# viscom-ulm/MCCNN

Measured on AMD Instinct MI355X. Metric: MC-convolved points/sec (fwd+bwd), 100k-pt cloud r=0.1, higher is better.
Workload: dtype f32; 1 GPU; ScanNet-like non-uniform room, 100000 pts/room, 1 room(s) on rank 0, absolute radius 0.1, KDE window 0.2, same-level conv 1to64 (Fin=1, Fout=64, combin), avg on; points_total=100000, points_per_gpu=100000, edges_per_gpu=4543198, layer=1to64, parallelism=cloud-per-GPU dp1, headline_mode=pipelined, rccl_world_size=1, collectives_warmed_before_warmup=False

## Files before the change

### mccnn_amd/MCConvModule.py

```python
import ctypes as C
import os
import threading
import time
import weakref

import numpy as _np
import torch

from . import _env, _lib
from ._lib import check, ptr, stream_handle


class InvalidArgumentError(ValueError):
    pass


def _req(cond, msg):
    if not cond:
        raise InvalidArgumentError(msg)


def _f32(t, name):
    _req(isinstance(t, torch.Tensor) and t.is_cuda, "%s must be a CUDA tensor" % name)
    _req(t.dtype == torch.float32, "%s must be float32" % name)
# ... 355 lines not shown
    if e <= 500000:
        return True
    if not backward:
        return not (fin <= 128 and feats.shape[0] >= 65536)
    return fin >= 256 and e / float(rows) >= ROWS_MIN_DEGREE


def clear_caches():
    _ORDER_HINTS.clear()
    _WS_POOL.clear()
    _NUM_CELLS_CACHE.clear()
    _EDGE_GUESS.clear()
    _EDGE_RATIO.clear()


CHECK_BATCH_IDS = False


def check_batch_ids(inBatchIds, batchSize):
    bids = _i32(inBatchIds, "batch_ids")
    bad = torch.empty(1, dtype=torch.int32, device=bids.device)
    check(_lib.load().mccnn_check_batch_ids(ptr(bids), bids.shape[0], int(batchSize), ptr(bad), stream_handle()),
          "check_batch_ids")
    return int(bad.item())


_DEBUG_IMPL = 0


def debug_conv_impl(mask):
    global _DEBUG_IMPL
    prev = _DEBUG_IMPL
    _DEBUG_IMPL = int(mask)
    _lib.load().mccnn_debug_conv_impl(int(mask) & 3)
    return prev


def _num_cells(aabbMin, aabbMax, batchSize, cellSize, scaleInv):
    lib = _lib.load()
    if scaleInv:
        out = C.c_int(0)
        check(lib.mccnn_num_cells(None, None, batchSize, float(cellSize), 1, C.byref(out), None), "num_cells")
        return out.value
    key = (id(aabbMin), id(aabbMax))
    hit = _NUM_CELLS_CACHE.get(key)
    ext = None
    if hit is not None:
        rmin, rmax, vmin, vmax, val = hit
        if rmin() is aabbMin and rmax() is aabbMax and vmin == aabbMin._version and vmax == aabbMax._version:
            ext = val
    if ext is None:
        out = C.c_float(0.0)
        check(lib.mccnn_aabb_extent(ptr(aabbMin), ptr(aabbMax), C.byref(out), stream_handle()), "aabb_extent")
        ext = _np.float32(out.value)
        _evict_oldest(_NUM_CELLS_CACHE, 256)
        _NUM_CELLS_CACHE[key] = (weakref.ref(aabbMin), weakref.ref(aabbMax), aabbMin._version, aabbMax._version, ext)
    _req(cellSize > 0, "cell size must be positive")
    nc = int(ext / _np.float32(cellSize))
    return nc if nc != 0 else 1


def _seed_num_cells(aabbMin, aabbMax, extent):
    _evict_oldest(_NUM_CELLS_CACHE, 256)
    _NUM_CELLS_CACHE[(id(aabbMin), id(aabbMax))] = (weakref.ref(aabbMin), weakref.ref(aabbMax), aabbMin._version,
                                                    aabbMax._version, _np.float32(extent))


# ... 937 lines not shown
```

### mccnn_amd/_env.py

```python
import os
import sys

KNOWN_KEYS = (
    "small_off", "plan_small", "plan_small_max_l", "plan_mid_l", "plan_min_l", "rows_force",
    "rows_min_degree", "unsorted_max_points", "force_valu", "no_f1", "f1_x4_min_e", "f1_x4_waves_per_cu", "nw_lean",
    "nw_lds_pad", "scan_bg_tiles", "issue_thread", "job_delay_us",
    "hier_trace", "geo_own_pool", "trace_terminate", "aabb_one_max", "plan_batch_sync", "caller_join_off", "bwd_min_chunks",
    "fuse_sort", "native_prefetch", "plan_prefetch", "plan_prefetch_max_e", "geo_prefetch_min",
    "ecap_scale", "hier_pmode", "geo_trace")


def _parse():
    out = {}
    for item in os.environ.get("MCCNN_DEBUG", "").split(","):
        item = item.strip()
        if not item:
            continue
        k, _, v = item.partition("=")
        out[k.strip()] = v.strip() if _ else "1"
        if k.strip() not in KNOWN_KEYS:
            sys.stderr.write("mccnn: MCCNN_DEBUG key %r is not known (mccnn_amd/_env.py KNOWN_KEYS): ignored\n" % k.strip())
    return out


_OPTS = _parse()


def flag(name, default=True):
    v = os.environ.get("MCCNN_" + name)
    if v is None:
        return default
    return v != "0"


def debug(key, default, cast=None):
    v = _OPTS.get(key)
    if v is None:
        return default
    if cast is not None:
        return cast(v)
# ... 8 lines not shown
```

### mccnn_amd/csrc/conv.hip

```cpp
#include "conv_mfma.h"
#include "batch.h"
#include <cstdlib>
#include <type_traits>

namespace mccnn {

__device__ __forceinline__ float relu(float x) { return fmaxf(x, 0.0f); }
__device__ __forceinline__ float wave_sum(float v) {
#pragma unroll
    for (int d = 32; d >= 1; d >>= 1) v += __shfl_xor(v, d, 64);
    return v;
}

struct EdgeCtx {
    int j, i;
    float d0, d1, d2, inv;
};

__device__ __forceinline__ EdgeCtx load_edge(const ConvArgs& a, int t) {
    EdgeCtx c;
    int2 pr = a.packed[t];
    c.j = pr.x;
    c.i = pr.y;
    int b = clamp_batch(a.bids[c.j], a.B);
// ... 954 lines not shown
    if ((a.nb * 8) % Fin != 0) return MCCNN_E_SHAPE;
    a.outF = combin ? Fout : Fin;
    a.pts = sorted_pts; a.feats = sorted_feats; a.bids = sorted_batch_ids; a.pdfs = pdfs; a.samples = samples;
    a.start = start_idx; a.packed = reinterpret_cast<const int2*>(packed); a.mn = aabb_min; a.mx = aabb_max;
    a.w1 = w1; a.b1 = b1; a.w2 = w2; a.b2 = b2; a.w3 = w3; a.b3 = b3;
    a.n = n; a.m = m; a.e = e; a.Fin = Fin; a.Fout = Fout; a.radius = radius; a.invRadius = 1.0f / radius; a.scaleInv = scale_inv; a.avg = avg; a.B = batch_size;
    if (m > 0 && (!samples || !start_idx || !aabb_min || !aabb_max || !w1 || !b1 || !w2 || !b2 || !w3 || !b3))
        return MCCNN_E_BADARG;
    if (e > 0 && (!sorted_pts || !sorted_feats || !sorted_batch_ids || !pdfs || !packed)) return MCCNN_E_BADARG;
    return 0;
}

int launch_edge_records(const ConvArgs& a, float4* rec, hipStream_t s) {
    edge_records<<<ceil_div(a.e, 256), 256, 0, s>>>(a, rec);
    MCCNN_LAUNCHED();
    return 0;
}

void launch_reduce_partials(const float* partials, int rows, int nb, float* dw1, float* db1, float* dw2, float* db2,
                            float* dw3, float* db3, hipStream_t s) {
    reduce_partials<<<ceil_div((long long)nb * 176, 16), 1024, 0, s>>>(partials, rows, nb, dw1, db1, dw2, db2, dw3, db3, no_span());
}

int conv_fill_args(ConvArgs& a, const float* sorted_pts, const float* sorted_feats, const int* sorted_batch_ids,
                   const float* pdfs, const float* samples, const int* start_idx, const int* packed,
                   const float* aabb_min, const float* aabb_max, const float* w1, const float* b1, const float* w2,
                   const float* b2, const float* w3, const float* b3, int n, int m, int e, int Fin, int Fout, int combin,
                   int batch_size, float radius, int scale_inv, int avg) {
    return fill_args(a, sorted_pts, sorted_feats, sorted_batch_ids, pdfs, samples, start_idx, packed, aabb_min, aabb_max, w1,
                     b1, w2, b2, w3, b3, n, m, e, Fin, Fout, combin, batch_size, radius, scale_inv, avg);
}

std::atomic<int>& conv_impl_override() {
    static std::atomic<int> v{(debug_int("force_valu", 0) ? 1 : 0) | (debug_int("no_f1", 0) ? 2 : 0)};
    return v;
}

bool transpose_small(int e, int n) {
    return e <= MCCNN_TR_SMALL_E && n <= MCCNN_TR_SMALL_N && (long long)e * e / n <= (1LL << 20) && small_kernels_on();
}
size_t transpose_count_bytes(int n) { return align_up((size_t)n * 4) + scan_workspace_bytes(n); }
int transpose_count(const int2* pk, int e, int n, int* start_t, char* blk, int* slot, hipStream_t s) {
    const size_t cntBytes = align_up((size_t)n * 4);
    int* cnt = (int*)blk;
    {
        int rc = launch_clear_spans(clear_span(blk, cntBytes + scan_status_bytes(n)), no_span(), no_span(), s);
        if (rc) return rc;
    }
    if (n <= MCCNN_TR_LDS_BINS && e >= 4 * n) tr_count_lds<<<ceil_div(e, 256), 256, 0, s>>>(pk, e, n, cnt, slot);
    else tr_count<<<ceil_div(e, 256), 256, 0, s>>>(pk, e, cnt, slot);
    MCCNN_LAUNCHED();
    return exclusive_scan_i32(cnt, start_t, n, start_t + n, blk + cntBytes, s, true);
}
int transpose_fill(const int2* pk, int e, const int* start_t, const int* slot, int* tmp, hipStream_t s) {
    tr_fill<<<ceil_div(e, 256), 256, 0, s>>>(pk, e, start_t, slot, tmp);
    MCCNN_LAUNCHED();
    return 0;
}

}

using namespace mccnn;

template <bool TR>
static int launch_conv_stream(const ConvArgs& a, bool combin, bool vec, bool bf16, float* out, const float4* rec,
                              const int* permT, hipStream_t s, float4* recOut = nullptr) {
    typedef void (*Kern)(ConvArgs, float*, int, const float4*, const int*, float4*);
    Kern fn;
    if (bf16) fn = TR ? conv_stream<false, 4, true> : conv_stream<false, 4, false>;
    else if (TR) fn = vec ? conv_stream<false, 2, true> : conv_stream<false, 0, true>;
    else if (combin) fn = (a.Fin == 1) ? conv_stream<true, 1, false> : (a.Fin <= 4 ? conv_stream<true, 3, false> : conv_stream<true, 0, false>);
    else fn = vec ? conv_stream<false, 2, false> : conv_stream<false, 0, false>;
    const size_t lds = ((size_t)a.nb * MCCNN_WQ_FWD + 4 * (size_t)a.nb * 8) * sizeof(float);
    const int numCU = num_cus();
    const int perCU = cached_blocks_per_cu(reinterpret_cast<const void*>(fn), lds);
    const long long chunks = ((long long)a.e + 63) / 64;
    long long W = (long long)numCU * perCU * 4;
    if (W > (chunks + 1) / 2) W = (chunks + 1) / 2;
    if (W < 1) W = 1;
    fn<<<(int)((W + 3) / 4), 256, lds, s>>>(a, out, (int)W, rec, permT, recOut);
    MCCNN_LAUNCHED();
    return 0;
}

extern "C" {

int mccnn_debug_conv_impl(int mask) { return conv_impl_override().exchange(mask & 3); }

static bool f1_shape(int num_in_feats, int num_out_feats, int combin) {
    return combin && num_in_feats == 1 && num_out_feats > 0 && (num_out_feats + 7) / 8 <= MCCNN_LDS_MAX_NB &&
           (conv_impl_override().load(std::memory_order_relaxed) & 3) == 0;
}

static size_t state_record_bytes(int e) { return align_up((size_t)(e > 0 ? e : 0) * sizeof(float4)); }
size_t mccnn_spatial_conv_state_bytes(int m, int e, int num_in_feats, int num_out_feats, int combin) {
    if (m <= 0 || e <= 0 || num_in_feats <= 0 || num_out_feats <= 0) return 0;
    if (f1_shape(num_in_feats, num_out_feats, combin)) return state_record_bytes(e) + f1_state_bytes(m, (num_out_feats + 7) / 8);
    const long long neurons = combin ? (long long)num_in_feats * num_out_feats : num_in_feats;
    const bool mfma = (!combin || (neurons + 7) / 8 <= MCCNN_LDS_MAX_NB) && (conv_impl_override().load(std::memory_order_relaxed) & 1) == 0;
    return mfma ? state_record_bytes(e) : 0;
}

size_t mccnn_spatial_conv_fwd_workspace_bytes(int m, int e, int num_in_feats, int num_out_feats, int combin) {
    (void)e;
    if (m > 0 && f1_shape(num_in_feats, num_out_feats, combin)) return f1_fwd_workspace_bytes(m, (num_out_feats + 7) / 8);
    return 256;
}

static bool use_mfma(const ConvArgs& a, bool combin) {
    return (a.nb <= MCCNN_LDS_MAX_NB || !combin) && (conv_impl_override().load(std::memory_order_relaxed) & 1) == 0;
}
#define MCCNN_TILE_FWD 64
#define MCCNN_TILE_BWD 48
static void tile_split(int nb, int maxTile, int& tiles, int& per) {
    tiles = (nb + maxTile - 1) / maxTile;
    per = (nb + tiles - 1) / tiles;
}
static ConvArgs tile_args(const ConvArgs& a, int q0, int nbT, size_t elem) {
    ConvArgs t = a;
    t.feats = reinterpret_cast<const float*>(reinterpret_cast<const char*>(a.feats) + (size_t)q0 * 8 * elem);
// ... 336 lines not shown
```

### mccnn_amd/csrc/conv_f1.hip

```cpp
#include "conv_mfma.h"

namespace mccnn {

__device__ __forceinline__ float wave_seg_scan1(float v, float m1, float m2, float m4, float m8, float mA, float mB) {
    asm("s_nop 1\n"
        "v_fmac_f32_dpp %0, %0, %1 row_shr:1 row_mask:0xf bank_mask:0xf bound_ctrl:1\n s_nop 1\n"
        "v_fmac_f32_dpp %0, %0, %2 row_shr:2 row_mask:0xf bank_mask:0xf bound_ctrl:1\n s_nop 1\n"
        "v_fmac_f32_dpp %0, %0, %3 row_shr:4 row_mask:0xf bank_mask:0xf bound_ctrl:1\n s_nop 1\n"
        "v_fmac_f32_dpp %0, %0, %4 row_shr:8 row_mask:0xf bank_mask:0xf bound_ctrl:1\n s_nop 1\n"
        "v_fmac_f32_dpp %0, %0, %5 row_bcast:15 row_mask:0xa bank_mask:0xf\n s_nop 1\n"
        "v_fmac_f32_dpp %0, %0, %6 row_bcast:31 row_mask:0xc bank_mask:0xf\n s_nop 1\n"
        : "+v"(v)
        : "v"(m1), "v"(m2), "v"(m4), "v"(m8), "v"(mA), "v"(mB));
    return v;
}

__global__ __launch_bounds__(256) void f1_fwd_edges(ConvArgs a, float* __restrict__ A, float* __restrict__ S,
                                                    int numWaves, float4* __restrict__ recOut) {
    extern __shared__ float lds[];
    const int wave = threadIdx.x >> 6, lane = threadIdx.x & 63, i4 = lane & 3;
    const int rowA = a.nb * 8;
    float* wl = lds;
    float* carry = lds + a.nb * MCCNN_WQ_FWD + (size_t)wave * rowA;
    stage_weights<MCCNN_WQ_FWD>(a, wl);
// ... 464 lines not shown
                gb2[k] += t3[k];
            }
            float t4[8];
            MCCNN_PHASE();
            layer8<false>(w4 + 46, nullptr, i4, t3, t4);
            MCCNN_PHASE();
#pragma unroll
            for (int l = 0; l < 8; ++l) {
                float v = p1[l] ? t4[l] : 0.f;
                gw1[l * 3] = fmaf(v, rc.x, gw1[l * 3]);
                gw1[l * 3 + 1] = fmaf(v, rc.y, gw1[l * 3 + 1]);
                gw1[l * 3 + 2] = fmaf(v, rc.z, gw1[l * 3 + 2]);
                gb1[l] += v;
            }
        }
        {
            float r2 = wave_reduce64(gw2, lane);
            float misc[64];
#pragma unroll
            for (int k = 0; k < 24; ++k) misc[k] = gw1[k];
#pragma unroll
            for (int k = 0; k < 8; ++k) { misc[24 + k] = gb1[k]; misc[32 + k] = gb2[k]; }
#pragma unroll
            for (int k = 40; k < 64; ++k) misc[k] = 0.f;
            float rm = wave_reduce64(misc, lane);
            float* pq = prow + q * MCCNN_F1_ROW;
            pq[32 + lane] = r2;
            if (lane < 32) pq[lane] = rm;
            else if (lane < 40) pq[96 + lane - 32] = rm;
        }
    }
}

#define MCCNN_F1_ROWC 72
__global__ __launch_bounds__(256) void f1_bwd_centres(ConvArgs a, const float* __restrict__ outGrad,
                                                      const float* __restrict__ A, const float* __restrict__ S,
                                                      int cPerWave, int numSlices, float* __restrict__ G,
                                                      float* __restrict__ gb, float* __restrict__ partials,
                                                      float* __restrict__ featGrad) {
    for (long long i = (long long)blockIdx.x * blockDim.x + threadIdx.x; i < a.n; i += (long long)gridDim.x * blockDim.x)
        featGrad[i] = 0.f;
    const int wave = threadIdx.x >> 6, lane = threadIdx.x & 63;
    const int wid = blockIdx.x * 4 + wave;
    const int w = __builtin_amdgcn_readfirstlane(wid / (a.nb + 1));
    const int q = __builtin_amdgcn_readfirstlane(wid - w * (a.nb + 1));
    if (w >= numSlices) return;
    const int c0 = w * cPerWave;
    const int c1 = min(a.m, c0 + cPerWave);
    if (q == a.nb) {
        for (int i = c0 + lane; i < c1; i += 64) {
            const float* row = outGrad + (size_t)i * a.outF;
            float gbv = 0.f;
            int f = 0;
            if ((a.outF & 3) == 0) {
                for (; f + 4 <= a.outF; f += 4) {
                    const float4 gg = *reinterpret_cast<const float4*>(row + f);
                    gbv = fmaf(gg.x, a.b3[f], gbv);
                    gbv = fmaf(gg.y, a.b3[f + 1], gbv);
                    gbv = fmaf(gg.z, a.b3[f + 2], gbv);
                    gbv = fmaf(gg.w, a.b3[f + 3], gbv);
                }
            }
            for (; f < a.outF; ++f) gbv = fmaf(row[f], a.b3[f], gbv);
            gb[i] = gbv;
        }
        return;
// ... 74 lines not shown
            s2 += src[(size_t)(w + 128) * stride];
            s3 += src[(size_t)(w + 192) * stride];
        }
        for (; w < rows; w += 64) s0 += src[(size_t)w * stride];
    }
    acc[sl][kk] = (s0 + s1) + (s2 + s3);
    __syncthreads();
    if (sl == 0 && k < K) {
        float v = 0.f;
#pragma unroll
        for (int i = 0; i < 64; ++i) v += acc[i][kk];
        if (r < 24) dw1[q * 24 + r] = v;
        else if (r < 32) db1[q * 8 + r - 24] = v;
        else if (r < 96) dw2[q * 64 + r - 32] = v;
        else if (r < 104) db2[q * 8 + r - 96] = v;
        else if (r < 168) dw3[q * 64 + r - 104] = v;
        else db3[q * 8 + r - 168] = v;
    }
}

static void f1_bwd_partition(int e, int& cpw, int& waves) {
    const long long chunks = ((long long)e + 63) / 64;
    const long long resident = (long long)num_cus() * 4 * MCCNN_F1_OCC;
    cpw = (int)((chunks + resident - 1) / resident);
    if (cpw > 48) {
        const long long rounds = (cpw + 31) / 32;
        cpw = (int)((chunks + resident * rounds - 1) / (resident * rounds));
    }
    static const int minChunks = debug_int("bwd_min_chunks", 2);
    if (cpw < minChunks) cpw = minChunks < 1 ? 1 : minChunks;
    waves = (int)((chunks + cpw - 1) / cpw);
    if (waves < 1) waves = 1;
}
#ifndef MCCNN_F1_CENTRE_WAVES
#define MCCNN_F1_CENTRE_WAVES 1024
#endif
static void f1_centre_partition(int m, int& cPerWave, int& waves) {
    cPerWave = (m + MCCNN_F1_CENTRE_WAVES - 1) / MCCNN_F1_CENTRE_WAVES;
    cPerWave = (cPerWave + 63) / 64 * 64;
    waves = (m + cPerWave - 1) / cPerWave;
}

size_t f1_state_bytes(int m, int nb) { return align_up((size_t)m * nb * 8 * sizeof(float)) + align_up((size_t)m * sizeof(float)); }

static void f1_state_split(void* state, int m, int nb, float*& A, float*& S) {
    A = (float*)state;
    S = (float*)((char*)state + align_up((size_t)m * nb * 8 * sizeof(float)));
}

static int f1_run_edges(const ConvArgs& a, float* A, float* S, float4* recOut, hipStream_t s) {
    const size_t lds = ((size_t)a.nb * MCCNN_WQ_FWD + 4 * (size_t)a.nb * 8) * sizeof(float);
    if (a.e >= g_f1_x4_min_edges.load(std::memory_order_relaxed)) {
        const size_t lds4 = lds + 4 * 256 * sizeof(float4);
        const int perCU4 = cached_blocks_per_cu(reinterpret_cast<const void*>(f1_fwd_edges4), lds4);
        const long long iters = ((long long)a.e + 255) / 256;
        static const int wpc = debug_int("f1_x4_waves_per_cu", 0);
        long long W4 = (long long)num_cus() * (wpc > 0 ? wpc : perCU4 * 4);
        if (W4 > (iters + 1) / 2) W4 = (iters + 1) / 2;
        if (W4 < 1) W4 = 1;
        f1_fwd_edges4<<<(int)((W4 + 3) / 4), 256, lds4, s>>>(a, A, S, (int)W4, recOut);
        MCCNN_LAUNCHED();
        return 0;
    }
    const int perCU = cached_blocks_per_cu(reinterpret_cast<const void*>(f1_fwd_edges), lds);
    const long long chunks = ((long long)a.e + 63) / 64;
    long long W = (long long)num_cus() * perCU * 4;
    if (W > (chunks + 1) / 2) W = (chunks + 1) / 2;
    if (W < 1) W = 1;
    f1_fwd_edges<<<(int)((W + 3) / 4), 256, lds, s>>>(a, A, S, (int)W, recOut);
    MCCNN_LAUNCHED();
    return 0;
}

size_t f1_fwd_workspace_bytes(int m, int nb) { return f1_state_bytes(m, nb) + 256; }

int f1_forward(const ConvArgs& a, float* out, float4* rec_out, void* state, void* ws, size_t ws_bytes, hipStream_t s) {
    if (!state) {
        if (!ws || ws_bytes < f1_fwd_workspace_bytes(a.m, a.nb)) return MCCNN_E_WORKSPACE;
        state = ws;
    }
    float *A, *S;
    f1_state_split(state, a.m, a.nb, A, S);
    int rc = f1_run_edges(a, A, S, rec_out, s);
    if (rc) return rc;
    f1_fwd_centres<<<ceil_div((long long)a.m * a.nb, 256), 256, (size_t)a.nb * 72 * sizeof(float), s>>>(a, A, S, out);
    MCCNN_LAUNCHED();
    return 0;
}

size_t f1_bwd_workspace_bytes(int m, int e, int nb) {
    int cpw, wavesE, cpwC, wavesC;
    f1_bwd_partition(e, cpw, wavesE);
    f1_centre_partition(m, cpwC, wavesC);
    size_t b = f1_state_bytes(m, nb);
    b += align_up((size_t)m * nb * 8 * sizeof(float)) + align_up((size_t)m * sizeof(float));
    b += align_up((size_t)e * sizeof(float4)) + align_up((size_t)e * sizeof(float));
    b += align_up((size_t)(wavesE + 3) / 4 * 4 * nb * MCCNN_F1_ROW * sizeof(float));
    b += align_up((size_t)(wavesC + 3) / 4 * 4 * nb * MCCNN_F1_ROWC * sizeof(float));
    return b + 256;
}

int f1_backward(const ConvArgs& a, const float* out_grad, const float4* rec_in, const void* state, float* feat_grad, float* dw1, float* db1,
                float* dw2, float* db2, float* dw3, float* db3, void* ws, size_t ws_bytes, hipStream_t s) {
    if (!ws || ws_bytes < f1_bwd_workspace_bytes(a.m, a.e, a.nb)) return MCCNN_E_WORKSPACE;
    int cpw, wavesE, cPerWave, wavesC;
    f1_bwd_partition(a.e, cpw, wavesE);
    f1_centre_partition(a.m, cPerWave, wavesC);
    const int blocksE = (wavesE + 3) / 4, blocksC = (wavesC + 3) / 4;
    Arena ar(ws, ws_bytes);
    void* own = ar.take<char>(f1_state_bytes(a.m, a.nb));
    float* G = ar.take<float>((size_t)a.m * a.nb * 8);
    float* gb = ar.take<float>((size_t)a.m);
    float4* rec = ar.take<float4>((size_t)a.e);
    float* dfE = ar.take<float>((size_t)a.e);
    float* pe = ar.take<float>((size_t)blocksE * 4 * a.nb * MCCNN_F1_ROW);
    float* pc = ar.take<float>((size_t)blocksC * 4 * a.nb * MCCNN_F1_ROWC);
    if (!own || !G || !gb || !rec || !dfE || !pe || !pc) return MCCNN_E_WORKSPACE;
    float *A, *S;
    if (state) {
        f1_state_split(const_cast<void*>(state), a.m, a.nb, A, S);
    } else {
        f1_state_split(own, a.m, a.nb, A, S);
        int rc = f1_run_edges(a, A, S, nullptr, s);
        if (rc) return rc;
    }
    f1_bwd_centres<<<ceil_div((long long)wavesC * (a.nb + 1), 4), 256, 0, s>>>(a, out_grad, A, S, cPerWave, wavesC, G, gb, pc, feat_grad);
    MCCNN_LAUNCHED();
    const float4* recUse = rec;
    if (rec_in) {
        recUse = rec_in;
    } else {
        f1_edge_records<<<ceil_div(a.e, 256), 256, 0, s>>>(a, rec);
        MCCNN_LAUNCHED();
    }
    const size_t ldsE = (size_t)a.nb * MCCNN_WQ_BWD * sizeof(float);
    f1_bwd_edges<<<blocksE, 256, ldsE, s>>>(a, recUse, G, gb, feat_grad, dfE, cpw, pe);
    MCCNN_LAUNCHED();
    f1_reduce<<<ceil_div((long long)a.nb * 176, 16), 1024, 0, s>>>(pe, wavesE, pc, wavesC, a.nb, dw1, db1, dw2, db2, dw3, db3);
    MCCNN_LAUNCHED();
    return 0;
}

}
```

### mccnn_amd/csrc/conv_mfma.h

```cpp
#pragma once
#include "common.h"
#include <atomic>
#include <mutex>

namespace mccnn {

struct ConvArgs {
    const float* pts;
    const float* feats;
    const int* bids;
    const float* pdfs;
    const float* samples;
    const int* start;
    const int2* packed;
    const float* mn;
    const float* mx;
    const float *w1, *b1, *w2, *b2, *w3, *b3;
    int n, m, e, Fin, Fout, nb, neuronsOut, outF;
    float radius, invRadius;
    int scaleInv, avg, G, B;
};

#define MCCNN_LDS_MAX_NB 64
#define MCCNN_WQ_FWD 184
// ... 59 lines not shown
    if (BIAS) { bl = bias[i4]; bh = bias[4 + i4]; }
    f32x4 lo = {0.f, 0.f, 0.f, 0.f}, hi = lo;
#pragma unroll
    for (int k = 0; k < 8; ++k) {
        lo = MFMA4(al[k], x[k], lo);
        hi = MFMA4(ah[k], x[k], hi);
    }
    if (BIAS) {
        const float one = opaque_one();
        lo = MFMA4(bl, one, lo);
        hi = MFMA4(bh, one, hi);
    }
#pragma unroll
    for (int r = 0; r < 4; ++r) { y[r] = lo[r]; y[4 + r] = hi[r]; }
}

template <bool BIAS>
__device__ __forceinline__ void layer8_regs(const float* al, const float* ah, float bl, float bh, const float* x, float* y) {
    f32x4 lo = {0.f, 0.f, 0.f, 0.f}, hi = lo;
#pragma unroll
    for (int k = 0; k < 8; ++k) {
        lo = MFMA4(al[k], x[k], lo);
        hi = MFMA4(ah[k], x[k], hi);
    }
    if (BIAS) {
        const float one = opaque_one();
        lo = MFMA4(bl, one, lo);
        hi = MFMA4(bh, one, hi);
    }
#pragma unroll
    for (int r = 0; r < 4; ++r) { y[r] = lo[r]; y[4 + r] = hi[r]; }
}

struct BlockWeights {
    float w1lo[4], w1hi[4];
    float w2lo[8], w2hi[8], b2lo, b2hi;
    float w3lo[8], w3hi[8], b3lo, b3hi;
};
__device__ __forceinline__ void load_block_weights(const ConvArgs& a, int q, int i4, BlockWeights& w) {
    const int nl = q * 8 + i4, nh = nl + 4;
#pragma unroll
    for (int c = 0; c < 3; ++c) { w.w1lo[c] = a.w1[nl * 3 + c]; w.w1hi[c] = a.w1[nh * 3 + c]; }
    w.w1lo[3] = a.b1[nl]; w.w1hi[3] = a.b1[nh];
    const float4* r2l = reinterpret_cast<const float4*>(a.w2 + (size_t)q * 64 + i4 * 8);
    const float4* r2h = reinterpret_cast<const float4*>(a.w2 + (size_t)q * 64 + (4 + i4) * 8);
    const float4* r3l = reinterpret_cast<const float4*>(a.w3 + (size_t)q * 64 + i4 * 8);
    const float4* r3h = reinterpret_cast<const float4*>(a.w3 + (size_t)q * 64 + (4 + i4) * 8);
    const float4 a0 = r2l[0], a1 = r2l[1], b0 = r2h[0], b1 = r2h[1], c0 = r3l[0], c1 = r3l[1], d0 = r3h[0], d1 = r3h[1];
    w.w2lo[0] = a0.x; w.w2lo[1] = a0.y; w.w2lo[2] = a0.z; w.w2lo[3] = a0.w; w.w2lo[4] = a1.x; w.w2lo[5] = a1.y; w.w2lo[6] = a1.z; w.w2lo[7] = a1.w;
    w.w2hi[0] = b0.x; w.w2hi[1] = b0.y; w.w2hi[2] = b0.z; w.w2hi[3] = b0.w; w.w2hi[4] = b1.x; w.w2hi[5] = b1.y; w.w2hi[6] = b1.z; w.w2hi[7] = b1.w;
    w.w3lo[0] = c0.x; w.w3lo[1] = c0.y; w.w3lo[2] = c0.z; w.w3lo[3] = c0.w; w.w3lo[4] = c1.x; w.w3lo[5] = c1.y; w.w3lo[6] = c1.z; w.w3lo[7] = c1.w;
    w.w3hi[0] = d0.x; w.w3hi[1] = d0.y; w.w3hi[2] = d0.z; w.w3hi[3] = d0.w; w.w3hi[4] = d1.x; w.w3hi[5] = d1.y; w.w3hi[6] = d1.z; w.w3hi[7] = d1.w;
    w.b2lo = a.b2[nl]; w.b2hi = a.b2[nh];
    w.b3lo = a.b3[nl]; w.b3hi = a.b3[nh];
}
__device__ __forceinline__ void mlp_block_regs(const BlockWeights& w, float d0, float d1, float d2, float* a1, float* a2, float* o) {
    float pre[8];
    {
        f32x4 lo = {0.f, 0.f, 0.f, 0.f}, hi = lo;
        const float one = opaque_one();
        lo = MFMA4(w.w1lo[0], d0, lo);
        hi = MFMA4(w.w1hi[0], d0, hi);
        lo = MFMA4(w.w1lo[1], d1, lo);
        hi = MFMA4(w.w1hi[1], d1, hi);
        lo = MFMA4(w.w1lo[2], d2, lo);
        hi = MFMA4(w.w1hi[2], d2, hi);
        lo = MFMA4(w.w1lo[3], one, lo);
        hi = MFMA4(w.w1hi[3], one, hi);
#pragma unroll
        for (int r = 0; r < 4; ++r) { pre[r] = lo[r]; pre[4 + r] = hi[r]; }
    }
    MCCNN_PHASE();
#pragma unroll
    for (int r = 0; r < 8; ++r) a1[r] = relu1(pre[r]);
    MCCNN_PHASE();
    layer8_regs<true>(w.w2lo, w.w2hi, w.b2lo, w.b2hi, a1, pre);
    MCCNN_PHASE();
#pragma unroll
    for (int r = 0; r < 8; ++r) a2[r] = relu1(pre[r]);
    MCCNN_PHASE();
    layer8_regs<true>(w.w3lo, w.w3hi, w.b3lo, w.b3hi, a2, o);
    MCCNN_PHASE();
}

__device__ __forceinline__ void layer1_mfma(const f32x4* __restrict__ w, int i4, float d0, float d1, float d2, float* pre1) {
    f32x4 a1lo = w[i4], a1hi = w[4 + i4];
    f32x4 lo = {0.f, 0.f, 0.f, 0.f}, hi = lo;
    const float one = opaque_one();
    lo = MFMA4(a1lo.x, d0, lo);
    hi = MFMA4(a1hi.x, d0, hi);
    lo = MFMA4(a1lo.y, d1, lo);
    hi = MFMA4(a1hi.y, d1, hi);
    lo = MFMA4(a1lo.z, d2, lo);
    hi = MFMA4(a1hi.z, d2, hi);
    lo = MFMA4(a1lo.w, one, lo);
    hi = MFMA4(a1hi.w, one, hi);
#pragma unroll
    for (int r = 0; r < 4; ++r) { pre1[r] = lo[r]; pre1[4 + r] = hi[r]; }
}

__device__ __forceinline__ void mlp_block_l12(const float* __restrict__ wq, int i4, float d0, float d1, float d2,
                                              float* pre1, float* a1, float* pre2, float* a2) {
    const f32x4* w = reinterpret_cast<const f32x4*>(wq);
    layer1_mfma(w, i4, d0, d1, d2, pre1);
// ... 241 lines not shown
```

### mccnn_amd/csrc/debug_opts.h

```cpp
#pragma once
#include <cstdio>
#include <cstdlib>
#include <cstring>
#include <string>

namespace mccnn {

#define MCCNN_DEBUG_KEYS                                                                                                   \
    "small_off", "plan_small", "plan_small_max_l", "plan_mid_l", "plan_min_l", "rows_force",                              \
    "rows_min_degree", "unsorted_max_points", "force_valu", "no_f1", "f1_x4_min_e", "f1_x4_waves_per_cu", "nw_lean",      \
    "nw_lds_pad", "scan_bg_tiles", "issue_thread", "job_delay_us",                                                       \
    "hier_trace", "geo_own_pool", "trace_terminate", "aabb_one_max", "plan_batch_sync", "caller_join_off", "bwd_min_chunks", \
                                                                                    \
    "fuse_sort", "native_prefetch", "plan_prefetch", "plan_prefetch_max_e", "geo_prefetch_min",                          \
    "ecap_scale", "hier_pmode", "geo_trace"
static const char* const kDebugKeys[] = {MCCNN_DEBUG_KEYS};

inline const std::string& debug_list() {
    static const std::string list = [] {
        const char* e = getenv("MCCNN_DEBUG");
        std::string l(e ? e : "");
        size_t p = 0;
        while (p < l.size()) {
            size_t q = l.find(',', p);
            if (q == std::string::npos) q = l.size();
            size_t a = p, b = q;
            while (a < b && l[a] == ' ') ++a;
            while (b > a && l[b - 1] == ' ') --b;
            size_t eq = l.find('=', a);
            if (eq == std::string::npos || eq > b) eq = b;
            size_t kb = eq;
            while (kb > a && l[kb - 1] == ' ') --kb;
            const std::string key = l.substr(a, kb - a);
            if (!key.empty()) {
                bool known = false;
                for (const char* k : kDebugKeys) known = known || key == k;
                if (!known) fprintf(stderr, "mccnn: MCCNN_DEBUG key '%s' is not known (csrc/debug_opts.h kDebugKeys): ignored\n", key.c_str());
            }
            p = q + 1;
        }
        return l;
    }();
    return list;
}

// ... 24 lines not shown
```

### mccnn_amd/csrc/exec.hip

```cpp
#include "batch.h"

#include <chrono>
#include <cstdlib>
#include <cstring>
#include <new>
#include <thread>

namespace mccnn {
std::atomic<int>& conv_impl_override();
ClearSpan grid_head_span(int n, int batch_size, int num_cells, void* ws, size_t ws_bytes);
int build_grid_fused(const float* pts, const int* batch_ids, const float* aabb_min, const float* aabb_max, int n,
                     int batch_size, int num_cells, int* new_idx, float* out_pts, int* out_batch_ids, int* cell_indexs,
                     int* inv_idx, void* ws, size_t ws_bytes, hipStream_t s, const int* n_dev, bool cleared, ClearSpan x1,
                     ClearSpan x2);
size_t visiting_order_workspace_bytes(int m, int batch_size, int num_cells);
ClearSpan visiting_order_head_span(int m, int batch_size, int num_cells, void* ws, size_t ws_bytes);
int visiting_order(const float* pts, const int* batch_ids, const float* aabb_min, const float* aabb_max, int m, int batch_size,
                   int num_cells, int* order, void* ws, size_t ws_bytes, hipStream_t s, bool cleared);
bool plan_batchable(int rows, int e, int transposed);
size_t plan_batch_tr_ws_bytes(int n, int e);
int plan_batch_items(int transposed, const float* sorted_pts, const int* sorted_batch_ids, const float* pdfs, const float* samples,
                     const int* start_idx, const int* packed, const float* aabb_min, const float* aabb_max, int n, int m, int e,
                     int batch_size, float radius, int scale_inv, int avg, const int* order, int* start_t, int* perm_t,
                     int tlist_ready, void* plan_buffer, void* tws, size_t tws_bytes, TrSmallItem* tr, bool* use_tr,
// ... 77 lines not shown
        L.cells = o; o += al(cells_of(B, nc) * 8);
        L.new_idx = o; o += al(n1 * 4);
        L.inv_idx = o; o += al(n1 * 4);
    }
    L.start = o; o += al(m1 * 4);
    L.packed = o; o += al(e1 * 8);
    L.pdfs = o; o += al(e1 * 4);
    L.total = o; o += 256;
    L.order = o; o += al(m1 * 4);
    size_t w = mccnn_find_neighbors_workspace_bytes(m, n);
    size_t head = 0;
    if (with_grid) {
        const size_t g = mccnn_build_grid_workspace_bytes(n, B, nc);
        if (g == 0) return L;
        head += al(g);
    }
    if (m >= MCCNN_ORDER_MIN_M) {
        const size_t c = visiting_order_workspace_bytes(m, B, nc);
        if (c == 0) return L;
        head += al(c);
    }
    if (head > w) w = head;
    if (mccnn_sort_step1_workspace_bytes(m, B, nc) == 0) return L;
    const size_t p = mccnn_compute_pdf_workspace_bytes(e_cap, 1);
    if (p > w) w = p;
    if (max_neighbors > 0) w = al(w) + (mccnn_find_neighbors_capped_workspace_bytes(m, n) - mccnn_find_neighbors_workspace_bytes(m, n));
    L.ws = o;
    L.ws_bytes = al(w) + 256;
    o += L.ws_bytes;
    L.total_bytes = o;
    return L;
}

int read_mask() { return conv_impl_override().load(std::memory_order_relaxed); }

bool env_flag(const char* name, bool dflt) {
    const char* v = getenv(name);
    return v ? (strcmp(v, "0") != 0) : dflt;
}
bool row_kernels_on() { static const bool on = env_flag("MCCNN_ROW_KERNELS", true); return on; }
float rows_min_degree() { static const float d = (float)debug_float("rows_min_degree", 16.0); return d; }
int unsorted_max_points() { static const int v = debug_int("unsorted_max_points", 32768); return v; }

bool rows_shape(bool combin, int fin, const void* feats, int rows, int n_points, int e, bool backward) {
    if (!row_kernels_on() || read_mask() != 0 || combin || fin % 8 != 0 || e <= 0 || rows <= 0 || (((uintptr_t)feats) & 15)) return false;
    static const int force = debug_int("rows_force", 0);
    if (force == 1) return true;
    if (e <= 500000) return true;
    if (!backward) return !(fin <= 128 && n_points >= 65536);
    return fin >= 256 && (float)e / (float)rows >= rows_min_degree();
}

std::atomic<long long> g_wait_ns{0};

thread_local bool t_count_waits = true;

int wait_edges(mccnn_geometry* g, int spin_us) {
    if (g->e >= 0) return g->e;
    if (!g->total_host) return -1;
    int v = *g->total_host;
    if (v < 0 && spin_us != 0) {
        const auto t0 = std::chrono::steady_clock::now();
        struct Acc {
            std::chrono::steady_clock::time_point t;
            ~Acc() { if (t_count_waits) g_wait_ns.fetch_add(std::chrono::duration_cast<std::chrono::nanoseconds>(std::chrono::steady_clock::now() - t).count(), std::memory_order_relaxed); }
        } acc{t0};
        for (;;) {
// ... 972 lines not shown
```

Baseline: 171.8 million points/s.

## Add cooperative multi-wave F1 backward edge kernel sharing edge sweeps across waves

Adds a cooperative backward edge kernel for the Fin=1 combin path. W waves in a block each own one output-feature block per sweep, process the same edge chunk, and exchange per-edge feature-gradient partial sums through a small LDS buffer, so each edge's gradient accumulation is done cooperatively instead of each wave redoing it. It is selected when the edge count covers enough chunks per resident group. It also adds a per-edge barrier and extra register pressure from the per-wave gradient accumulators, and it repartitions the partials buffer. New debug mask bits control the path, and read_mask is masked so other code ignores them.

```diff
diff --git a/mccnn_amd/MCConvModule.py b/mccnn_amd/MCConvModule.py
--- a/mccnn_amd/MCConvModule.py
+++ b/mccnn_amd/MCConvModule.py
@@ -411,7 +411,7 @@
     global _DEBUG_IMPL
     prev = _DEBUG_IMPL
     _DEBUG_IMPL = int(mask)
-    _lib.load().mccnn_debug_conv_impl(int(mask) & 3)
+    _lib.load().mccnn_debug_conv_impl((int(mask) & 3) | 16)
     return prev
 
 
diff --git a/mccnn_amd/_env.py b/mccnn_amd/_env.py
--- a/mccnn_amd/_env.py
+++ b/mccnn_amd/_env.py
@@ -6,6 +6,7 @@
     "rows_min_degree", "unsorted_max_points", "force_valu", "no_f1", "f1_x4_min_e", "f1_x4_waves_per_cu", "nw_lean",
     "nw_lds_pad", "scan_bg_tiles", "issue_thread", "job_delay_us",
     "hier_trace", "geo_own_pool", "trace_terminate", "aabb_one_max", "plan_batch_sync", "caller_join_off", "bwd_min_chunks",
+    "f1_coop_min_chunks", "f1_coop_off", "f1_coop_force",
     "fuse_sort", "native_prefetch", "plan_prefetch", "plan_prefetch_max_e", "geo_prefetch_min",
     "ecap_scale", "hier_pmode", "geo_trace")
 
diff --git a/mccnn_amd/csrc/conv.hip b/mccnn_amd/csrc/conv.hip
--- a/mccnn_amd/csrc/conv.hip
+++ b/mccnn_amd/csrc/conv.hip
@@ -1010,7 +1010,8 @@
 }
 
 std::atomic<int>& conv_impl_override() {
-    static std::atomic<int> v{(debug_int("force_valu", 0) ? 1 : 0) | (debug_int("no_f1", 0) ? 2 : 0)};
+    static std::atomic<int> v{(debug_int("force_valu", 0) ? 1 : 0) | (debug_int("no_f1", 0) ? 2 : 0) |
+                              (debug_int("f1_coop_off", 0) ? 4 : 0) | (debug_int("f1_coop_force", 0) ? 8 : 0)};
     return v;
 }
 
@@ -1063,7 +1064,13 @@
 
 extern "C" {
 
-int mccnn_debug_conv_impl(int mask) { return conv_impl_override().exchange(mask & 3); }
+int mccnn_debug_conv_impl(int mask) {
+    std::atomic<int>& v = conv_impl_override();
+    if (!(mask & 16)) return v.exchange(mask & 15);
+    int old = v.load(std::memory_order_relaxed);
+    while (!v.compare_exchange_weak(old, (mask & 3) | (old & 12))) {}
+    return old;
+}
 
 static bool f1_shape(int num_in_feats, int num_out_feats, int combin) {
     return combin && num_in_feats == 1 && num_out_feats > 0 && (num_out_feats + 7) / 8 <= MCCNN_LDS_MAX_NB &&
diff --git a/mccnn_amd/csrc/conv_f1.hip b/mccnn_amd/csrc/conv_f1.hip
--- a/mccnn_amd/csrc/conv_f1.hip
+++ b/mccnn_amd/csrc/conv_f1.hip
@@ -520,6 +520,137 @@
     }
 }
 
+template <class T>
+__device__ __forceinline__ T ld_off32(const void* base, unsigned byteOff) {
+    return *reinterpret_cast<const T*>(reinterpret_cast<const char*>(base) + byteOff);
+}
+template <int W>
+__global__ __launch_bounds__(W * 64, MCCNN_F1_OCC) void f1_bwd_edges_coop(ConvArgs a, const float4* __restrict__ rec,
+                                                       const float* __restrict__ G, const float* __restrict__ gb,
+                                                       float* __restrict__ featGrad, float* __restrict__ dfE, int cpg,
+                                                       float* __restrict__ partials) {
+    __shared__ float xch[2][W][64];
+    const int wave = __builtin_amdgcn_readfirstlane(threadIdx.x >> 6), lane = threadIdx.x & 63, i4 = lane & 3;
+    const long long eBegL = (long long)blockIdx.x * cpg * 64;
+    if (eBegL >= a.e) return;
+    const int eBeg = (int)eBegL;
+    const int eEnd = (int)min((long long)a.e, eBegL + (long long)cpg * 64);
+    const int trips = (eEnd - eBeg + 63) >> 6;
+    const int sweeps = a.nb / W;
+    const unsigned tLast = (unsigned)a.e - 1u;
+    int parity = 0;
+
+    for (int s = 0; s < sweeps; ++s) {
+        const int q = s * W + wave;
+        const bool first = (s == 0), last = (s == sweeps - 1);
+        BwdBlockWeights wr;
+        load_bwd_block_weights(a, q, i4, wr);
+        const float* Gq = G + (size_t)q * a.m * 8;
+        float gw2[64], gb2[8], gw1[24], gb1[8];
+#pragma unroll
+        for (int k = 0; k < 64; ++k) gw2[k] = 0.f;
+#pragma unroll
+        for (int k = 0; k < 8; ++k) { gb2[k] = 0.f; gb1[k] = 0.f; }
+#pragma unroll
+        for (int k = 0; k < 24; ++k) gw1[k] = 0.f;
+
+        int2 prN;
+        float4 rcN;
+        {
+            const unsigned t0 = min((unsigned)(eBeg + lane), tLast);
+            prN = ld_off32<int2>(a.packed, t0 * 8u);
+            rcN = ld_off32<float4>(rec, t0 * 16u);
+        }
+        for (int k = 0; k < trips; ++k) {
+            const int t = eBeg + k * 64 + lane;
+            const bool act = t < eEnd;
+            const bool own = (k & (W - 1)) == wave;
+            const int2 pr = prN;
+            const float4 rc = rcN;
+            const int j = pr.x, ci = pr.y;
+            const float inv = act ? rc.w : 0.f;
+            const float4 g0 = ld_off32<float4>(Gq, (unsigned)ci * 32u), g1 = ld_off32<float4>(Gq, (unsigned)ci * 32u + 16u);
+            const float f = ld_off32<float>(a.feats, (unsigned)j * 4u);
+            float tot = 0.f, gbi = 0.f;
+            if (own) {
+#ifndef MCCNN_F1_COOP_SWEEP_ATOMIC
+                if (act && !first) tot = dfE[t];
+#endif
+                if (last) gbi = ld_off32<float>(gb, (unsigned)ci * 4u);
+            }
+            {
+                const unsigned tn = min((unsigned)t + 64u, tLast);
+                prN = ld_off32<int2>(a.packed, tn * 8u);
+                rcN = ld_off32<float4>(rec, tn * 16u);
+            }
+            const float Gv[8] = {g0.x, g0.y, g0.z, g0.w, g1.x, g1.y, g1.z, g1.w};
+            const float sE = f * inv;
+            float a1[8], a2[8];
+            bool p1[8], p2[8];
+            {
+                float pre1[8], pre2[8];
+                mlp_block_l12_regs(wr, rc.x, rc.y, rc.z, pre1, a1, pre2, a2);
+#pragma unroll
+                for (int r = 0; r < 8; ++r) { p1[r] = pre1[r] >= 0.0f; p2[r] = pre2[r] >= 0.0f; }
+            }
+            float sfg = 0.f;
+#pragma unroll
+            for (int r = 0; r < 8; ++r) sfg = fmaf(Gv[r], a2[r], sfg);
+            xch[parity][wave][lane] = sfg;
+            float t3[8];
+#pragma unroll
+            for (int r = 0; r < 8; ++r) t3[r] = p2[r] ? Gv[r] * sE : 0.f;
+#pragma unroll
+            for (int r = 0; r < 8; ++r) {
+#pragma unroll
+                for (int l = 0; l < 8; ++l) gw2[r * 8 + l] = fmaf(t3[r], a1[l], gw2[r * 8 + l]);
+                gb2[r] += t3[r];
+            }
+            float t4[8];
+            MCCNN_PHASE();
+            layer8_regs<false>(wr.w2tlo, wr.w2thi, 0.f, 0.f, t3, t4);
+            MCCNN_PHASE();
+#pragma unroll
+            for (int l = 0; l < 8; ++l) {
+                const float v = p1[l] ? t4[l] : 0.f;
+                gw1[l * 3] = fmaf(v, rc.x, gw1[l * 3]);
+                gw1[l * 3 + 1] = fmaf(v, rc.y, gw1[l * 3 + 1]);
+                gw1[l * 3 + 2] = fmaf(v, rc.z, gw1[l * 3 + 2]);
+                gb1[l] += v;
+            }
+            __syncthreads();
+            if (own) {
+#pragma unroll
+                for (int w = 0; w < W; ++w) tot += xch[parity][w][lane];
+                if (act) {
+#ifdef MCCNN_F1_COOP_SWEEP_ATOMIC
+                    atomicAdd(&featGrad[j], (tot + gbi) * inv);
+#else
+                    if (last) atomicAdd(&featGrad[j], (tot + gbi) * inv);
+                    else dfE[t] = tot;
+#endif
+                }
+            }
+            parity ^= 1;
+        }
+        {
+            float r2 = wave_reduce64(gw2, lane);
+            float misc[64];
+#pragma unroll
+            for (int k = 0; k < 24; ++k) misc[k] = gw1[k];
+#pragma unroll
+            for (int k = 0; k < 8; ++k) { misc[24 + k] = gb1[k]; misc[32 + k] = gb2[k]; }
+#pragma unroll
+            for (int k = 40; k < 64; ++k) misc[k] = 0.f;
+            float rm = wave_reduce64(misc, lane);
+            float* pq = partials + ((size_t)blockIdx.x * a.nb + q) * MCCNN_F1_ROW;
+            pq[32 + lane] = r2;
+            if (lane < 32) pq[lane] = rm;
+            else if (lane < 40) pq[96 + lane - 32] = rm;
+        }
+    }
+}
+
 #define MCCNN_F1_ROWC 72
 __global__ __launch_bounds__(256) void f1_bwd_centres(ConvArgs a, const float* __restrict__ outGrad,
                                                       const float* __restrict__ A, const float* __restrict__ S,
@@ -660,6 +791,34 @@
     waves = (int)((chunks + cpw - 1) / cpw);
     if (waves < 1) waves = 1;
 }
+static int f1_coop_width(int nb) { return nb % 8 == 0 ? 8 : nb % 4 == 0 ? 4 : nb % 2 == 0 ? 2 : 0; }
+static long long f1_coop_resident(int W) { return (long long)num_cus() * 4 * MCCNN_F1_OCC / W; }
+static void f1_coop_partition(int e, int W, int& cpg, int& groups) {
+    const long long chunks = ((long long)e + 63) / 64;
+    const long long resident = f1_coop_resident(W);
+    cpg = (int)((chunks + resident - 1) / resident);
+    if (cpg > 48 * W) {
+        const long long rounds = (cpg + 32 * W - 1) / (32 * W);
+        cpg = (int)((chunks + resident * rounds - 1) / (resident * rounds));
+    }
+    static const int minChunks = debug_int("bwd_min_chunks", 2);
+    if (cpg < minChunks) cpg = minChunks < 1 ? 1 : minChunks;
+    groups = (int)((chunks + cpg - 1) / cpg);
+    if (groups < 1) groups = 1;
+}
+static bool f1_coop_fits(int n, int m, int e) { return e < (1 << 27) && m < (1 << 26) && n < (1 << 29); }
+#ifndef MCCNN_F1_COOP_MIN_CHUNKS
+#define MCCNN_F1_COOP_MIN_CHUNKS 3
+#endif
+static int f1_coop_choice(int n, int m, int e, int nb) {
+    const int W = f1_coop_width(nb);
+    const int mask = conv_impl_override().load(std::memory_order_relaxed);
+    if (W == 0 || (mask & 4) || !f1_coop_fits(n, m, e)) return 0;
+    if (mask & 8) return W;
+    static const int minChunks = debug_int("f1_coop_min_chunks", MCCNN_F1_COOP_MIN_CHUNKS);
+    const long long chunks = ((long long)e + 63) / 64;
+    return chunks >= f1_coop_resident(W) * minChunks ? W : 0;
+}
 #ifndef MCCNN_F1_CENTRE_WAVES
 #define MCCNN_F1_CENTRE_WAVES 1024
 #endif
@@ -723,7 +882,13 @@
     size_t b = f1_state_bytes(m, nb);
     b += align_up((size_t)m * nb * 8 * sizeof(float)) + align_up((size_t)m * sizeof(float));
     b += align_up((size_t)e * sizeof(float4)) + align_up((size_t)e * sizeof(float));
-    b += align_up((size_t)(wavesE + 3) / 4 * 4 * nb * MCCNN_F1_ROW * sizeof(float));
+    size_t rowsE = (size_t)(wavesE + 3) / 4 * 4;
+    if (const int W = f1_coop_width(nb)) {
+        int cpg, groups;
+        f1_coop_partition(e, W, cpg, groups);
+        if ((size_t)groups > rowsE) rowsE = (size_t)groups;
+    }
+    b += align_up(rowsE * nb * MCCNN_F1_ROW * sizeof(float));
     b += align_up((size_t)(wavesC + 3) / 4 * 4 * nb * MCCNN_F1_ROWC * sizeof(float));
     return b + 256;
 }
@@ -735,13 +900,17 @@
     f1_bwd_partition(a.e, cpw, wavesE);
     f1_centre_partition(a.m, cPerWave, wavesC);
     const int blocksE = (wavesE + 3) / 4, blocksC = (wavesC + 3) / 4;
+    const int coopW = f1_coop_choice(a.n, a.m, a.e, a.nb);
+    int cpg = 0, groups = 0;
+    if (coopW) f1_coop_partition(a.e, coopW, cpg, groups);
+    const size_t rowsE = (size_t)groups > (size_t)blocksE * 4 ? (size_t)groups : (size_t)blocksE * 4;
     Arena ar(ws, ws_bytes);
     void* own = ar.take<char>(f1_state_bytes(a.m, a.nb));
     float* G = ar.take<float>((size_t)a.m * a.nb * 8);
     float* gb = ar.take<float>((size_t)a.m);
     float4* rec = ar.take<float4>((size_t)a.e);
     float* dfE = ar.take<float>((size_t)a.e);
-    float* pe = ar.take<float>((size_t)blocksE * 4 * a.nb * MCCNN_F1_ROW);
+    float* pe = ar.take<float>(rowsE * a.nb * MCCNN_F1_ROW);
     float* pc = ar.take<float>((size_t)blocksC * 4 * a.nb * MCCNN_F1_ROWC);
     if (!own || !G || !gb || !rec || !dfE || !pe || !pc) return MCCNN_E_WORKSPACE;
     float *A, *S;
@@ -761,10 +930,15 @@
         f1_edge_records<<<ceil_div(a.e, 256), 256, 0, s>>>(a, rec);
         MCCNN_LAUNCHED();
     }
-    const size_t ldsE = (size_t)a.nb * MCCNN_WQ_BWD * sizeof(float);
-    f1_bwd_edges<<<blocksE, 256, ldsE, s>>>(a, recUse, G, gb, feat_grad, dfE, cpw, pe);
+    if (coopW == 8) f1_bwd_edges_coop<8><<<groups, 512, 0, s>>>(a, recUse, G, gb, feat_grad, dfE, cpg, pe);
+    else if (coopW == 4) f1_bwd_edges_coop<4><<<groups, 256, 0, s>>>(a, recUse, G, gb, feat_grad, dfE, cpg, pe);
+    else if (coopW == 2) f1_bwd_edges_coop<2><<<groups, 128, 0, s>>>(a, recUse, G, gb, feat_grad, dfE, cpg, pe);
+    else {
+        const size_t ldsE = (size_t)a.nb * MCCNN_WQ_BWD * sizeof(float);
+        f1_bwd_edges<<<blocksE, 256, ldsE, s>>>(a, recUse, G, gb, feat_grad, dfE, cpw, pe);
+    }
     MCCNN_LAUNCHED();
-    f1_reduce<<<ceil_div((long long)a.nb * 176, 16), 1024, 0, s>>>(pe, wavesE, pc, wavesC, a.nb, dw1, db1, dw2, db2, dw3, db3);
+    f1_reduce<<<ceil_div((long long)a.nb * 176, 16), 1024, 0, s>>>(pe, coopW ? groups : wavesE, pc, wavesC, a.nb, dw1, db1, dw2, db2, dw3, db3);
     MCCNN_LAUNCHED();
     return 0;
 }
diff --git a/mccnn_amd/csrc/conv_mfma.h b/mccnn_amd/csrc/conv_mfma.h
--- a/mccnn_amd/csrc/conv_mfma.h
+++ b/mccnn_amd/csrc/conv_mfma.h
@@ -115,6 +115,55 @@
     for (int r = 0; r < 4; ++r) { y[r] = lo[r]; y[4 + r] = hi[r]; }
 }
 
+__device__ __forceinline__ void layer1_regs(const float* lo4, const float* hi4, float d0, float d1, float d2, float* pre1) {
+    f32x4 lo = {0.f, 0.f, 0.f, 0.f}, hi = lo;
+    const float one = opaque_one();
+    lo = MFMA4(lo4[0], d0, lo);
+    hi = MFMA4(hi4[0], d0, hi);
+    lo = MFMA4(lo4[1], d1, lo);
+    hi = MFMA4(hi4[1], d1, hi);
+    lo = MFMA4(lo4[2], d2, lo);
+    hi = MFMA4(hi4[2], d2, hi);
+    lo = MFMA4(lo4[3], one, lo);
+    hi = MFMA4(hi4[3], one, hi);
+#pragma unroll
+    for (int r = 0; r < 4; ++r) { pre1[r] = lo[r]; pre1[4 + r] = hi[r]; }
+}
+
+struct BwdBlockWeights {
+    float w1lo[4], w1hi[4];
+    float w2lo[8], w2hi[8], b2lo, b2hi;
+    float w2tlo[8], w2thi[8];
+};
+__device__ __forceinline__ void load_bwd_block_weights(const ConvArgs& a, int q, int i4, BwdBlockWeights& w) {
+    const int nl = q * 8 + i4, nh = nl + 4;
+#pragma unroll
+    for (int c = 0; c < 3; ++c) { w.w1lo[c] = a.w1[nl * 3 + c]; w.w1hi[c] = a.w1[nh * 3 + c]; }
+    w.w1lo[3] = a.b1[nl]; w.w1hi[3] = a.b1[nh];
+    const float* w2 = a.w2 + (size_t)q * 64;
+    const float4* r2l = reinterpret_cast<const float4*>(w2 + i4 * 8);
+    const float4* r2h = reinterpret_cast<const float4*>(w2 + (4 + i4) * 8);
+    const float4 a0 = r2l[0], a1 = r2l[1], b0 = r2h[0], b1 = r2h[1];
+    w.w2lo[0] = a0.x; w.w2lo[1] = a0.y; w.w2lo[2] = a0.z; w.w2lo[3] = a0.w; w.w2lo[4] = a1.x; w.w2lo[5] = a1.y; w.w2lo[6] = a1.z; w.w2lo[7] = a1.w;
+    w.w2hi[0] = b0.x; w.w2hi[1] = b0.y; w.w2hi[2] = b0.z; w.w2hi[3] = b0.w; w.w2hi[4] = b1.x; w.w2hi[5] = b1.y; w.w2hi[6] = b1.z; w.w2hi[7] = b1.w;
+    w.b2lo = a.b2[nl]; w.b2hi = a.b2[nh];
+#pragma unroll
+    for (int k = 0; k < 8; ++k) { w.w2tlo[k] = w2[k * 8 + i4]; w.w2thi[k] = w2[k * 8 + 4 + i4]; }
+}
+__device__ __forceinline__ void mlp_block_l12_regs(const BwdBlockWeights& w, float d0, float d1, float d2,
+                                                   float* pre1, float* a1, float* pre2, float* a2) {
+    layer1_regs(w.w1lo, w.w1hi, d0, d1, d2, pre1);
+    MCCNN_PHASE();
+#pragma unroll
+    for (int r = 0; r < 8; ++r) a1[r] = relu1(pre1[r]);
+    MCCNN_PHASE();
+    layer8_regs<true>(w.w2lo, w.w2hi, w.b2lo, w.b2hi, a1, pre2);
+    MCCNN_PHASE();
+#pragma unroll
+    for (int r = 0; r < 8; ++r) a2[r] = relu1(pre2[r]);
+    MCCNN_PHASE();
+}
+
 struct BlockWeights {
     float w1lo[4], w1hi[4];
     float w2lo[8], w2hi[8], b2lo, b2hi;
@@ -139,20 +188,7 @@
 }
 __device__ __forceinline__ void mlp_block_regs(const BlockWeights& w, float d0, float d1, float d2, float* a1, float* a2, float* o) {
     float pre[8];
-    {
-        f32x4 lo = {0.f, 0.f, 0.f, 0.f}, hi = lo;
-        const float one = opaque_one();
-        lo = MFMA4(w.w1lo[0], d0, lo);
-        hi = MFMA4(w.w1hi[0], d0, hi);
-        lo = MFMA4(w.w1lo[1], d1, lo);
-        hi = MFMA4(w.w1hi[1], d1, hi);
-        lo = MFMA4(w.w1lo[2], d2, lo);
-        hi = MFMA4(w.w1hi[2], d2, hi);
-        lo = MFMA4(w.w1lo[3], one, lo);
-        hi = MFMA4(w.w1hi[3], one, hi);
-#pragma unroll
-        for (int r = 0; r < 4; ++r) { pre[r] = lo[r]; pre[4 + r] = hi[r]; }
-    }
+    layer1_regs(w.w1lo, w.w1hi, d0, d1, d2, pre);
     MCCNN_PHASE();
 #pragma unroll
     for (int r = 0; r < 8; ++r) a1[r] = relu1(pre[r]);
diff --git a/mccnn_amd/csrc/debug_opts.h b/mccnn_amd/csrc/debug_opts.h
--- a/mccnn_amd/csrc/debug_opts.h
+++ b/mccnn_amd/csrc/debug_opts.h
@@ -11,6 +11,7 @@
     "rows_min_degree", "unsorted_max_points", "force_valu", "no_f1", "f1_x4_min_e", "f1_x4_waves_per_cu", "nw_lean",      \
     "nw_lds_pad", "scan_bg_tiles", "issue_thread", "job_delay_us",                                                       \
     "hier_trace", "geo_own_pool", "trace_terminate", "aabb_one_max", "plan_batch_sync", "caller_join_off", "bwd_min_chunks", \
+    "f1_coop_min_chunks", "f1_coop_off", "f1_coop_force",                                                                \
                                                                                     \
     "fuse_sort", "native_prefetch", "plan_prefetch", "plan_prefetch_max_e", "geo_prefetch_min",                          \
     "ecap_scale", "hier_pmode", "geo_trace"
diff --git a/mccnn_amd/csrc/exec.hip b/mccnn_amd/csrc/exec.hip
--- a/mccnn_amd/csrc/exec.hip
+++ b/mccnn_amd/csrc/exec.hip
@@ -133,7 +133,7 @@
     return L;
 }
 
-int read_mask() { return conv_impl_override().load(std::memory_order_relaxed); }
+int read_mask() { return conv_impl_override().load(std::memory_order_relaxed) & 3; }
 
 bool env_flag(const char* name, bool dflt) {
     const char* v = getenv(name);
```

New measurement: 177.8 million points/s, median of 6. +3.5%, better.
